# jzhoubu/vsearch

Hardware: AMD Instinct MI355X
Metric: queries/sec over 21M-doc sparse index, k=100; recall@100 vs reference (higher is better)
Workload: dtype f32

## Files before the change

vsearch_amd/csrc/bp_quad.h:

```cpp
#pragma once
#include "bp_walk.h"
#include "bp_quad_loop.h"
#include "bp_quad_asm.h"

#ifndef VS_QUAD_EPI
#define VS_QUAD_EPI 2
#endif

namespace vs {

constexpr int kQuadRows = 2048;
constexpr int kQuadQT = 8;
constexpr int kQuadPer = kBpEntCap / kScanThreads;
constexpr size_t kQuadAccBytes = (size_t)(kQuadRows / 16) * kQuadGroupDw * 4;
static_assert(kBpEntCap % kScanThreads == 0, "a thread owns a fixed number of entries");
static_assert(kQuadAccBytes >= kBpSortBytes, "the accumulator area holds the 8192-slot entry sort");
__host__ __device__ constexpr size_t quad_fixed_lds() { return kQuadAccBytes + (size_t)kBpCap * 8 + (size_t)kQuadQT * 16 + 64 * 4; }
__host__ __device__ constexpr size_t quad_cut_lds() { return quad_fixed_lds() + (size_t)(kBpEntCap + 64 + 64 * kQuadOverRead) * 8; }
__host__ __device__ constexpr size_t quad_lds_bytes() { return quad_cut_lds() + (size_t)kCutHistWords * 4; }
static_assert(quad_lds_bytes() <= (size_t)160 * 1024, "the quad walk's LDS");
static_assert(kBpCap == 2 * kScanThreads, "wg_cut_topk: two keys of the candidate buffer a thread");
static_assert(kQuadQT == 8 && (kQuadAccBytes + (size_t)kBpCap * 8) % 16 == 0, "the epilogue reads thresholds and counters 16 bytes at a time");
constexpr int kQuadListCap = 64 - 4 * kQuadOverRead, kQuadListBytes = (kQuadListCap + 4 * kQuadOverRead) * 8;
static_assert(kQuadListCap >= 16, "room for links in a wave's list");
static_assert(2 * kQuadListBytes * kScanWaves <= kBpCap * 8, "the link lists fit the sort buffer");
constexpr int kQuadLinked = kQuadCells - 2;
constexpr double kQuadMaxRatio = 3.0;
constexpr int kQuadPaceDefault = 0;
template <int CELLS, int LINKED>
__host__ __device__ constexpr uint32_t chunk_overflow(uint32_t n) { return n > (uint32_t)CELLS ? (n - (uint32_t)CELLS + (uint32_t)LINKED - 1u) / (uint32_t)LINKED : 0u; }
__host__ __device__ constexpr uint32_t quad_overflow_chunks(uint32_t n) { return chunk_overflow<kQuadCells, kQuadLinked>(n); }

template <int CELLS, int LINKED>
__global__ __launch_bounds__(kScanThreads) void quad_count_kernel(const uint32_t* pk_ptr, const uint4* cols, int64_t n_rows, int32_t n_cols, int32_t rows,
                                                                  uint32_t* dir, uint32_t* block_recs, unsigned long long* df_rec, unsigned long long* df_nnz,
                                                                  int32_t* overflow) {
    extern __shared__ __attribute__((aligned(16))) char smem[];
    uint32_t* cnt = reinterpret_cast<uint32_t*>(smem);
    __shared__ int scratch[32];
    const int tid = threadIdx.x;
    const int64_t n_blocks = (n_rows + rows - 1) / rows;
    const int seg = (n_cols + kScanThreads - 1) / kScanThreads;
    for (int64_t b = blockIdx.x; b < n_blocks; b += gridDim.x) {
        const int64_t r0 = b * rows, r1 = min(n_rows, r0 + rows);
        const uint32_t P0 = pk_ptr[r0], P1 = pk_ptr[r1];
        __syncthreads();
        for (int i = tid; i <= n_cols; i += kScanThreads) cnt[i] = 0;
        __syncthreads();
        for (uint32_t p = P0 + tid; p < P1; p += kScanThreads) {
            const uint4 cw = cols[p];
            const uint32_t cwv[4] = {cw.x, cw.y, cw.z, cw.w};
#pragma unroll
            for (int i = 0; i < 4; ++i) {
                atomicAdd(&cnt[cwv[i] & 0xFFFFu], 1u);
                atomicAdd(&cnt[cwv[i] >> 16], 1u);
            }
        }
        __syncthreads();
        const int i0 = min(n_cols, tid * seg), i1 = min(n_cols, i0 + seg);
        int mine = 0;
        for (int i = i0; i < i1; ++i) mine += (int)chunk_overflow<CELLS, LINKED>(cnt[i]);
        int tot = 0;
        int off = block_excl_scan(mine, scratch, tid, &tot);
        uint32_t* d = dir + (size_t)b * (n_cols + 1);
        for (int i = i0; i < i1; ++i) {
            const uint32_t c = cnt[i], r = chunk_overflow<CELLS, LINKED>(c);
            d[i] = bp_dir_pack((uint32_t)off, r);
            if (r > kBpDirRecMask || (uint32_t)off > kBpDirUnitMax) overflow[0] = 1;
            off += (int)r;
            atomicAdd(&df_rec[i], (unsigned long long)(1u + r));
            if (c) atomicAdd(&df_nnz[i], (unsigned long long)c);
        }
        if (tid == 0) { d[n_cols] = bp_dir_pack((uint32_t)tot, 0u); block_recs[b] = (uint32_t)n_cols + (uint32_t)tot; }
    }
}

template <int VS>
__global__ __launch_bounds__(kScanThreads) void quad_fill_kernel(const uint32_t* pk_ptr, const uint4* cols, const void* vals, int64_t n_rows, int32_t n_cols,
                                                                 int32_t rows, const uint32_t* dir, const unsigned long long* base, uint32_t* rec) {
    extern __shared__ __attribute__((aligned(16))) char smem[];
    uint32_t* cur = reinterpret_cast<uint32_t*>(smem);
    const int tid = threadIdx.x, lane = tid & 63, w = tid >> 6;
    const int64_t n_blocks = (n_rows + rows - 1) / rows;
    for (int64_t b = blockIdx.x; b < n_blocks; b += gridDim.x) {
        const int64_t r0 = b * rows, r1 = min(n_rows, r0 + rows);
        const uint32_t* d = dir + (size_t)b * (n_cols + 1);
        __syncthreads();
        for (int i = tid; i <= n_cols; i += kScanThreads) cur[i] = 0u;
        __syncthreads();
        uint32_t* brec = rec + (size_t)base[b] * kQuadCells;
        for (int64_t r = r0 + w; r < r1; r += kScanWaves) {
            const uint32_t p0 = pk_ptr[r], p1 = pk_ptr[r + 1];
            const uint32_t ai = quad_acc_index((uint32_t)(r - r0));
            for (uint32_t p = p0 + lane; p < p1; p += 64) {
                const uint4 cw = cols[p];
                const uint32_t cwv[4] = {cw.x, cw.y, cw.z, cw.w};
                uint32_t hb[8];
                if constexpr (VS == VM_F32) {
                    const float4* vp = reinterpret_cast<const float4*>(vals);
                    const float4 v0 = vp[2 * (size_t)p], v1 = vp[2 * (size_t)p + 1];
                    const float v[8] = {v0.x, v0.y, v0.z, v0.w, v1.x, v1.y, v1.z, v1.w};
#pragma unroll
                    for (int i = 0; i < 8; ++i) hb[i] = (uint32_t)__half_as_ushort(__float2half_rn(v[i]));
                } else {
                    const uint4 hv = reinterpret_cast<const uint4*>(vals)[p];
                    const uint32_t h4[4] = {hv.x, hv.y, hv.z, hv.w};
#pragma unroll
                    for (int i = 0; i < 8; ++i) hb[i] = (i & 1) ? (h4[i >> 1] >> 16) : (h4[i >> 1] & 0xFFFFu);
                }
#pragma unroll
// ... 36 lines not shown
        __syncthreads();
        for (int i = tid; i < nc * 16; i += 256) {
            const uint4 v = src[i];
            uint32_t* q = in + (i >> 4) * LD + (i & 15) * 4;
            q[0] = v.x; q[1] = v.y; q[2] = v.z; q[3] = v.w;
        }
        __syncthreads();
        if (tid < nc) {
            const uint32_t* mi = in + tid * LD;
            uint32_t* mo = out + tid * LD;
            uint32_t mask[4] = {0u, 0u, 0u, 0u}, fill[4] = {0u, 0u, 0u, 0u}, room[4] = {16u, 16u, 16u, 16u};
            const bool linked = (mi[63] >> 31) != 0u;
            if (linked) {
                mo[62] = mi[62]; mo[63] = mi[63];
                mask[2] |= 1u << (mi[62] & 31u); mask[3] |= 1u << (mi[63] & 31u);
                room[2] = 15u; room[3] = 15u;
            }
            for (int i = 0; i < (linked ? kQuadLinked : kQuadCells); ++i) {
                const uint32_t p = mi[i];
                if ((p & 0x7FFF0000u) == 0u) continue;
                const uint32_t bit = 1u << (p & 31u);
                int pick = -1, any = -1;
                uint32_t best = 17u, best_any = 17u;
#pragma unroll
                for (int j = 0; j < 4; ++j) {
                    if (fill[j] < room[j] && fill[j] < best_any) { best_any = fill[j]; any = j; }
                    if (fill[j] < room[j] && !(mask[j] & bit) && fill[j] < best) { best = fill[j]; pick = j; }
                }
                if (pick < 0) pick = any;
#pragma unroll
                for (int j = 0; j < 4; ++j)
                    if (j == pick) { mo[fill[j] * 4 + j] = p; mask[j] |= bit; ++fill[j]; }
            }
#pragma unroll
            for (int j = 0; j < 4; ++j)
                while (fill[j] < room[j]) {
                    const uint32_t freeb = ~mask[j];
                    const uint32_t bk = freeb ? (uint32_t)(__ffs((int)freeb) - 1) : 0u;
                    mo[fill[j] * 4 + j] = quad_acc_index(bk);
                    mask[j] |= 1u << bk;
                    ++fill[j];
                }
        }
        __syncthreads();
        uint4* dst = reinterpret_cast<uint4*>(rec + c0 * kQuadCells);
        for (int i = tid; i < nc * 16; i += 256) {
            const uint32_t* q = out + (i >> 4) * LD + (i & 15) * 4;
            dst[i] = make_uint4(q[0], q[1], q[2], q[3]);
        }
    }
}

typedef unsigned short quad_us2 __attribute__((ext_vector_type(2)));

static_assert(kQuadRows <= 2 * kScanThreads && kQuadQT * 2 <= 32, "a thread's filter bits: two document rounds x the slots in one word");
constexpr int kQuadFiltWords = kQuadRows / 32 + 1;
constexpr size_t kQuadFiltStageBytes = (size_t)kQuadFiltWords * kQuadQT * 4;
static_assert(kQuadFiltWords * kQuadQT <= kScanThreads && quad_lds_bytes() + kQuadFiltStageBytes <= (size_t)160 * 1024, "the per-query filter stage");
template <int TM, int FL = 0>
__global__ __launch_bounds__(kScanThreads) void bp_quad_topk(KArg<BpArgs, FL> a) {
    constexpr int QT = kQuadQT;
    extern __shared__ __attribute__((aligned(16))) char smem[];
    int32_t* acc = reinterpret_cast<int32_t*>(smem);
    uint64_t* sortbuf = reinterpret_cast<uint64_t*>(smem + kQuadAccBytes);
    unsigned long long* tau = reinterpret_cast<unsigned long long*>(sortbuf + kBpCap);
    unsigned long long* upper_sh = tau + QT;
    int* scratch = reinterpret_cast<int*>(upper_sh + QT);
    unsigned int* ccnt = reinterpret_cast<unsigned int*>(scratch + 48);
    unsigned int* chi = ccnt + QT;
    uint2* desc = reinterpret_cast<uint2*>(scratch + 64);
    const uint32_t desc_lds = (uint32_t)quad_fixed_lds();
    uint32_t* cut_hist = reinterpret_cast<uint32_t*>(smem + quad_cut_lds());

    const int tid = threadIdx.x, lane = tid & 63, wv = tid >> 6;
    const int K = a.k;
    uint64_t* my_gcand = a.gcand + (size_t)blockIdx.x * QT * kBpCap;
    const int64_t n_blocks = (a.n_rows + a.rows - 1) / a.rows;
    const int64_t items = (int64_t)(a.n_tiles_dev ? a.n_tiles_dev[0] : a.n_tiles) * a.nchunk;
    const unsigned long long k_rt0 = TM ? __builtin_amdgcn_s_memrealtime() : 0ull;
    auto lds_barrier = [&]() { asm volatile("s_waitcnt lgkmcnt(0)\n\ts_barrier" ::: "memory"); };
    const uint32_t list_a = (uint32_t)kQuadAccBytes + (uint32_t)wv * 2u * kQuadListBytes, list_b = list_a + kQuadListBytes;
    const uint32_t g8 = (uint32_t)(lane >> 4) * 8u, s16 = (uint32_t)(lane & 15) * 16u;

    for (int64_t item = blockIdx.x; item < items; item += gridDim.x) {
        const int tile = (int)(item / a.nchunk), c = (int)(item % a.nchunk);
        const int q0 = a.tiles[tile].x, nq = a.tiles[tile].y;
        [[maybe_unused]] long long tm = TM ? (long long)__builtin_readcyclecounter() : 0;
        [[maybe_unused]] uint32_t tacc[6] = {0u, 0u, 0u, 0u, 0u, 0u};
        auto lap = [&](int phase) {
            if constexpr (TM != 0) {
                const long long now = (long long)__builtin_readcyclecounter();
                tacc[phase] += (uint32_t)(now - tm);
                tm = now;
            }
        };
        const int64_t b0 = (int64_t)c * a.blocks_per_chunk, b1 = min(n_blocks, b0 + a.blocks_per_chunk);
        __syncthreads();
        const int64_t e0 = a.qptr[q0], e1 = a.qptr[q0 + nq];
        const int n_ent = (int)(e1 - e0);
        const int n_static = (n_ent + 63) & ~63;
        {
            uint64_t* skey = reinterpret_cast<uint64_t*>(acc);
            for (int i = tid; i < 8192; i += kScanThreads) {
                uint64_t key = 0;
                if (i < n_ent) {
                    const int64_t e = e0 + i;
                    int qs = 0;
                    while (e >= a.qptr[q0 + qs + 1]) ++qs;
                    const float w = a.qvals[e] * a.qscale[q0 + qs];
                    key = ((uint64_t)1 << 63) | ((uint64_t)(uint32_t)a.qcols[e] << 40) | ((uint64_t)qs << 32) | (uint64_t)__float_as_uint(w);
                }
                skey[i] = key;
            }
            wg_sort_desc<kScanThreads>(skey, 8192, tid);
            for (int i = tid; i < n_static + 64 * kQuadOverRead; i += kScanThreads) {
                uint2 dsc = make_uint2(0u, 0u);
                if (i < n_ent) {
                    const uint64_t key = skey[i];
                    const uint32_t col = (uint32_t)(key >> 40) & 0xFFFFu, qs = (uint32_t)(key >> 32) & 0xFFu;
                    dsc = make_uint2((col << 8) | (qs * 16u), (uint32_t)key);
                }
                desc[i] = dsc;
            }
            __syncthreads();
        }
        for (int i = tid; i < (int)(kQuadAccBytes / 4); i += kScanThreads) acc[i] = 0;
        if (tid < QT) { tau[tid] = 0ull; ccnt[tid] = 0u; chi[tid] = 0u; }
        if (tid < QT) upper_sh[tid] = (a.upper && tid < nq) ? a.upper[q0 + tid] : ~0ull;
        __syncthreads();
        const uint32_t trips = (uint32_t)(n_static / 64);
        bool pace_off = false;
        unsigned long long base_cur = b0 < b1 ? a.base[b0] : 0ull;
        for (int64_t b = b0; b < b1 || b == b0; ++b) {
            const bool have = b < b1;
            const int rows_b = have ? (int)min((int64_t)a.rows, a.n_rows - b * a.rows) : 0;
            [[maybe_unused]] uint32_t fw0 = 0u, fw1 = 0u;
            if constexpr (FL != 0) {
                if (a.filt.ld == 0) {
                    const uint64_t bit = (uint64_t)(a.filt.bit0 + b * a.rows + tid);
                    if (tid < rows_b) fw0 = a.filt.words[bit >> 5];
                    if (tid + kScanThreads < rows_b) fw1 = a.filt.words[(bit + kScanThreads) >> 5];
                } else if (have) {
                    const int64_t w0 = (a.filt.bit0 + b * a.rows) >> 5, w1 = (a.filt.bit0 + b * a.rows + rows_b - 1) >> 5;
                    const int q = tid & (QT - 1), w = tid / QT;
                    if (w < kQuadFiltWords && q < nq && w0 + w <= w1) fw0 = a.filt.words[(size_t)(q0 + q) * (size_t)a.filt.ld + (size_t)(w0 + w)];
                }
            }
            if (have && trips > 0) {
                const char* brec = a.rec + (size_t)base_cur * kQuadChunkBytes;
                auto chain = [&](uint32_t n, uint32_t cur, uint32_t nxt) {
                    for (int depth = 0; n > 0 && depth < kQuadRows / kQuadLinked + 2; ++depth) {
                        const uint32_t n_pad = (n + 3u) & ~3u;
                        if ((uint32_t)lane < n_pad - n + 4u * kQuadOverRead)
                            reinterpret_cast<uint2*>(smem + cur)[n + (uint32_t)lane] = make_uint2(0u, 0u);
                        asm volatile("s_waitcnt lgkmcnt(0)" ::: "memory");
                        n = quad_list_asm(cur + g8, n_pad / 4u, brec, s16, nxt, (uint32_t)kQuadListCap);
                        const uint32_t t = cur; cur = nxt; nxt = t;
                    }
                };
                const uint32_t n_link = quad_walk_asm(desc_lds + (uint32_t)wv * 32u + g8, trips, brec, s16, list_a, (uint32_t)kQuadListCap);
                if (n_link <= (uint32_t)kQuadListCap) {
                    chain(n_link, list_a, list_b);
                } else {
                    constexpr uint32_t kSeg = kQuadListCap / 4;
                    for (uint32_t t0 = 0; t0 < trips; t0 += kSeg) {
                        const uint32_t n = quad_collect_asm(desc_lds + (uint32_t)wv * 32u + g8 + t0 * 512u, min(kSeg, trips - t0), brec, s16, list_a, (uint32_t)kQuadListCap);
                        chain(n, list_a, list_b);
                    }
                }
            }
            lap(1);
            if (a.pace && items <= (int64_t)gridDim.x && tid == 0 && have && !pace_off) {
                uint32_t* pc = a.pace + (size_t)c * a.blocks_per_chunk;
                const int64_t rel = b - b0;
                if (!((a.knob & 64) && blockIdx.x == 0))
                    __hip_atomic_fetch_add(pc + rel, 1u, __ATOMIC_RELAXED, __HIP_MEMORY_SCOPE_AGENT);
                if (rel >= a.pace_window) {
                    const uint32_t need = (uint32_t)(items / a.nchunk);
                    if (!pace_wait(pc + rel - a.pace_window, need)) pace_off = true;
                }
            }
            if (b + 1 < b1) base_cur = a.base[b + 1];
            if (a.gtau && tid < nq) { const unsigned long long g = a.gtau[q0 + tid]; if (g > tau[tid]) tau[tid] = g; }
            [[maybe_unused]] uint32_t fbits = 0u;
            [[maybe_unused]] uint32_t* fstage = reinterpret_cast<uint32_t*>(smem + quad_lds_bytes());
            if constexpr (FL != 0) {
                if (a.filt.ld == 0) {
#pragma unroll
                    for (int r = 0; r < 2; ++r) {
                        const uint64_t bit = (uint64_t)(a.filt.bit0 + b * a.rows + r * kScanThreads + tid);
                        if (r * kScanThreads + tid < rows_b && (((r ? fw1 : fw0) >> (bit & 31u)) & 1u)) fbits |= 0xFFu << (r * QT);
                    }
                } else if (tid < kQuadFiltWords * QT) {
                    fstage[tid] = fw0;
                }
                __builtin_amdgcn_s_waitcnt(0x0F70);
            }
            lds_barrier();
            if constexpr (FL != 0) {
                if (a.filt.ld != 0) {
                    const int64_t w0 = (a.filt.bit0 + b * a.rows) >> 5;
#pragma unroll
                    for (int r = 0; r < 2; ++r) {
                        const int d = r * kScanThreads + tid;
                        if (d < rows_b) {
                            const uint64_t bit = (uint64_t)(a.filt.bit0 + b * a.rows + d);
                            const uint4* p = reinterpret_cast<const uint4*>(fstage + ((int64_t)(bit >> 5) - w0) * QT);
                            const uint4 lo = p[0], hi = p[1];
                            const uint32_t w[QT] = {lo.x, lo.y, lo.z, lo.w, hi.x, hi.y, hi.z, hi.w};
#pragma unroll
                            for (int q = 0; q < QT; ++q) fbits |= ((w[q] >> (bit & 31u)) & 1u) << (r * QT + q);
                        }
                    }
                }
            }
            uint32_t pf = 0;
            if ((a.knob & 512) == 0 && b + 1 < b1 && (uint32_t)(lane >> 3) < trips) {
                const uint32_t dx = *reinterpret_cast<const uint32_t*>(smem + desc_lds + (uint32_t)(lane >> 3) * 512u + (uint32_t)wv * 32u + (uint32_t)((lane >> 1) & 3) * 8u);
                const char* pl = a.rec + (size_t)base_cur * kQuadChunkBytes + (dx & 0xFFFFFF00u) + (uint32_t)(lane & 1) * 128u;
                asm volatile("global_load_dword %0, %1, off" : "=v"(pf) : "v"(pl) : "memory");
            }
            lap(2);
            int32_t thr[QT];
            bool thr_stale = true;
            for (int d0 = 0; d0 < rows_b || d0 == 0; d0 += kScanThreads) {
                const int d = d0 + tid;
                const bool more = d0 + kScanThreads < rows_b;
                const uint32_t inc = more ? 1u : 0x10000u;
                if (d0 == 0 || thr_stale) {
                    const uint4* t4 = reinterpret_cast<const uint4*>(tau);
#pragma unroll
                    for (int i = 0; i < QT / 2; ++i) {
                        const uint4 t = t4[i];
                        thr[2 * i] = 2 * i < nq ? (int32_t)(t.y ^ 0x80000000u) : 0x7FFFFFFF;
                        thr[2 * i + 1] = 2 * i + 1 < nq ? (int32_t)(t.w ^ 0x80000000u) : 0x7FFFFFFF;
                    }
                    thr_stale = false;
                }
                if (d < rows_b) {
                    const int64_t row = b * a.rows + d;
                    int32_t sums[QT];
#if VS_QUAD_EPI == 0
                    int32_t* pa = acc + quad_acc_index((uint32_t)d);
#pragma unroll
                    for (int q = 0; q < QT; ++q) sums[q] = pa[q * 16];
#pragma unroll
                    for (int q = 0; q < QT; ++q) pa[q * 16] = 0;
#elif VS_QUAD_EPI == 1
                    {
                        const uint32_t pa = quad_acc_index((uint32_t)d) * 4u, zero = 0u;
                        asm volatile("ds_wrxchg_rtn_b32 %0, %8, %9\n\tds_wrxchg_rtn_b32 %1, %8, %9 offset:64\n\tds_wrxchg_rtn_b32 %2, %8, %9 offset:128\n\t"
                                     "ds_wrxchg_rtn_b32 %3, %8, %9 offset:192\n\tds_wrxchg_rtn_b32 %4, %8, %9 offset:256\n\tds_wrxchg_rtn_b32 %5, %8, %9 offset:320\n\t"
                                     "ds_wrxchg_rtn_b32 %6, %8, %9 offset:384\n\tds_wrxchg_rtn_b32 %7, %8, %9 offset:448\n\ts_waitcnt lgkmcnt(0)"
                                     : "=&v"(sums[0]), "=&v"(sums[1]), "=&v"(sums[2]), "=&v"(sums[3]), "=&v"(sums[4]), "=&v"(sums[5]), "=&v"(sums[6]), "=&v"(sums[7])
                                     : "v"(pa), "v"(zero) : "memory");
                    }
#else
                    {
                        const uint32_t pa = quad_acc_index((uint32_t)d) * 4u, zero = 0u;
                        unsigned long long s01, s23, s45, s67;
                        asm volatile("ds_wrxchg2_rtn_b32 %0, %4, %5, %5 offset0:0 offset1:16\n\tds_wrxchg2_rtn_b32 %1, %4, %5, %5 offset0:32 offset1:48\n\t"
                                     "ds_wrxchg2_rtn_b32 %2, %4, %5, %5 offset0:64 offset1:80\n\tds_wrxchg2_rtn_b32 %3, %4, %5, %5 offset0:96 offset1:112\n\ts_waitcnt lgkmcnt(0)"
                                     : "=&v"(s01), "=&v"(s23), "=&v"(s45), "=&v"(s67) : "v"(pa), "v"(zero) : "memory");
                        sums[0] = (int32_t)(uint32_t)s01; sums[1] = (int32_t)(uint32_t)(s01 >> 32); sums[2] = (int32_t)(uint32_t)s23; sums[3] = (int32_t)(uint32_t)(s23 >> 32);
                        sums[4] = (int32_t)(uint32_t)s45; sums[5] = (int32_t)(uint32_t)(s45 >> 32); sums[6] = (int32_t)(uint32_t)s67; sums[7] = (int32_t)(uint32_t)(s67 >> 32);
                    }
#endif
#pragma unroll
                    for (int q = 0; q < QT; ++q) {
                        if (sums[q] >= thr[q] && (FL == 0 || ((fbits >> ((d0 >= kScanThreads ? QT : 0) + q)) & 1u) != 0u)) {
                            const uint32_t hi = (uint32_t)sums[q] ^ 0x80000000u;
                            const uint64_t key = ((uint64_t)hi << 32) | (uint32_t)(~(uint32_t)row);
                            if (key > tau[q] && key < upper_sh[q]) {
                                const uint32_t old = atomicAdd(&ccnt[q], inc);
                                my_gcand[(size_t)q * kBpCap + (old & 0xFFFFu) + (old >> 16)] = key;
                            }
                        }
                    }
                }
                static_assert(kQuadRows <= 2 * kScanThreads, "the cut counter has two fields, first rounds | last round: a block is at most two epilogue rounds");
                lds_barrier();
                if ((a.knob & 128) && __builtin_amdgcn_readfirstlane(wv) == 5)
                    for (int i = 0; i < (a.knob >> 12); ++i) __builtin_amdgcn_s_sleep(8);
                const bool last = b + 1 >= b1 && !more;
                uint32_t cmax;
                {
                    const uint4* c4 = reinterpret_cast<const uint4*>(ccnt);
                    const uint4 c0 = c4[0], c1 = c4[1];
                    const uint32_t w[QT] = {c0.x, c0.y, c0.z, c0.w, c1.x, c1.y, c1.z, c1.w};
                    uint32_t t[QT];
                    if (more) {
                        const uint4 h0 = c4[2], h1 = c4[3];
                        const uint32_t h[QT] = {h0.x, h0.y, h0.z, h0.w, h1.x, h1.y, h1.z, h1.w};
#pragma unroll
                        for (int q = 0; q < QT; ++q) t[q] = __builtin_amdgcn_udot2(__builtin_bit_cast(quad_us2, w[q]), quad_us2{1, 0}, h[q], false);
                    } else {
#pragma unroll
                        for (int q = 0; q < QT; ++q) t[q] = __builtin_amdgcn_udot2(__builtin_bit_cast(quad_us2, w[q]), quad_us2{1, 1}, 0u, false);
                        if (tid < QT) chi[tid] = ccnt[tid] >> 16;
                    }
                    cmax = max(max(max(t[0], t[1]), max(t[2], t[3])), max(max(t[4], t[5]), max(t[6], t[7])));
                }
                const bool any = last || cmax > (uint32_t)(kBpCap - kScanThreads);
                [[maybe_unused]] long long t_cut = 0;
                if constexpr (TM != 0) t_cut = (long long)__builtin_readcyclecounter();
                if (any) __syncthreads();
                thr_stale = any;
                if (any)
                for (int qs = 0; qs < nq; ++qs) {
                    const uint32_t cw = ccnt[qs], cnt = (cw & 0xFFFFu) + (more ? chi[qs] : (cw >> 16));
                    if (last || cnt > (uint32_t)(kBpCap - kScanThreads)) {
                        for (int i = tid; i < kBpCap; i += kScanThreads) sortbuf[i] = (uint32_t)i < cnt ? my_gcand[(size_t)qs * kBpCap + i] : 0ull;
                        if (last) {
                            uint64_t* out = a.cand + ((size_t)(q0 + qs) * a.nchunk + c) * (size_t)K;
                            if (K <= 256) {
                                wg_final_topk256<kScanThreads>(sortbuf, cnt, K, my_gcand + (size_t)qs * kBpCap, out, cut_hist, tid);
                            } else {
                                wg_sort_desc<kScanThreads>(sortbuf, kBpCap, tid);
                                for (int i = tid; i < K; i += kScanThreads) out[i] = sortbuf[i];
                            }
                        } else if (cnt > (uint32_t)K) {
                            const unsigned long long kth_sel = wg_cut_topk<kScanThreads>(sortbuf, K, my_gcand + (size_t)qs * kBpCap, cut_hist, tid);
                            if (tid == 0) {
                                const unsigned long long kth = kth_sel;
                                if (kth > tau[qs]) tau[qs] = kth;
                                if (a.gtau && kth != 0ull) atomicMax(a.gtau + q0 + qs, kth);
                                ccnt[qs] = (uint32_t)K;
                                chi[qs] = 0u;
                            }
                        }
                        __syncthreads();
                    }
                }
                if constexpr (TM != 0) { if (any) tacc[3] += (uint32_t)((long long)__builtin_readcyclecounter() - t_cut); }
            }
            asm volatile("s_waitcnt vmcnt(0)" : "+v"(pf) : : "memory");
            lap(4);
            if constexpr (TM != 0) tacc[5] += 1u;
            if (b + 1 >= b1) break;
        }
        if constexpr (TM != 0) {
            if ((tid & 63) == 0) {
#pragma unroll
                for (int i = 0; i < 6; ++i) atomicAdd(a.timing + i, (unsigned long long)tacc[i]);
            }
        }
    }
    if (TM && threadIdx.x == 0) {
        a.timing[16 + 4 * blockIdx.x] = __builtin_amdgcn_s_memrealtime() - k_rt0;
        a.timing[17 + 4 * blockIdx.x] = k_rt0;
        a.timing[18 + 4 * blockIdx.x] = (unsigned long long)__builtin_amdgcn_s_getreg((3 << 11) | 20);
        a.timing[19 + 4 * blockIdx.x] = (unsigned long long)__builtin_amdgcn_s_getreg((31 << 11) | 4);
    }
}

}
```

vsearch_amd/csrc/bp_search.hip:

```cpp
#include "csr_internal.h"
#include "bp_refine.h"
#include "bp_bin.h"
#include "bp_quad.h"
#include "bp_head.h"
#include "bp_bq.h"

#include <chrono>
#include <vector>

namespace vs {


bool bp_wanted(const vs_index* idx) {
    if (idx->bp_pref == 0 || idx->n_rows <= 0 || idx->n_packets <= 0) return false;
    if (((size_t)idx->n_cols + 1) * 4 + 4096 > 160 * 1024) return false;
    if (idx->bp_pref == 1) return true;
    if (idx->store_dtype == VS_NONE) return idx->n_rows >= 65536;
    return idx->n_rows >= 16384 && (double)idx->nnz / (double)idx->n_rows >= 256.0;
}

void bp_release(vs_index* idx) {
    idx->bp_dir.release(); idx->bp_base.release(); idx->bp_rec.release(); idx->bp_df.release(); idx->bp_vmax.release();
    idx->bp_hmap.release(); idx->bp_strip.release();
    idx->bp_n_head = 0;
// ... 436 lines not shown
                       bq_pk ? idx->bp_bq_maxrow : 0, bq_pk ? flag16 : (uint32_t*)nullptr);
    if (bq_pk) hipLaunchKernelGGL(bq_split_kernel<0>, dim3(1), dim3(kScanThreads), 0, s, (const int2*)tiles, reinterpret_cast<const int32_t*>(dplan), (const uint32_t*)flag16,
                                  tiles16, tiles2, n_split);
    VS_HIP(hipGetLastError());
    VS_STAGE("sparsify", s);
    const bool head_gemm = idx->bp_n_head > 0 && idx->bp_head_gemm;
    int tiles_per_pass = 0, n_pass = 1;
    const int head_ks = bp_head_pad(idx->bp_n_head) / 32;
    if (head_gemm) {
        const size_t per_tile = (size_t)n_blocks * (size_t)idx->bp_rows * 8 * 2;
        size_t free_b = 0, total_b = 0;
        VS_HIP(hipMemGetInfo(&free_b, &total_b));
        DevBuf& head_out = device_scratch(idx->device, kScratchHeadOut);
        DevBuf& head_w = device_scratch(idx->device, kScratchHeadW);
        const size_t have = head_out.bytes, margin = (size_t)6 << 30;
        const size_t room = std::min<size_t>(free_b + have > margin ? free_b + have - margin : 0, total_b / 4);
        static const int tpp_env = getenv("VS_HEAD_TILES") ? atoi(getenv("VS_HEAD_TILES")) : 0;
        int tpp = (int)std::min<size_t>(std::max<size_t>(have, std::min<size_t>(room, (size_t)48 << 30)) / std::max<size_t>(per_tile, 1), (size_t)ceil_div(B, qt));
        if (tpp_env > 0) tpp = std::min(tpp, tpp_env);
        if (idx->bp_head_tiles > 0) tpp = std::min(tpp, idx->bp_head_tiles);
        if (tpp >= 64) tpp = tpp / 64 * 64;
        else if (tpp >= 2) tpp &= ~1;
        if (tpp < 1) return fail(VS_ENOMEM, "head pre-pass: no HBM for the dense sums of one tile (%.2f GB)", (double)per_tile / 1e9);
        tiles_per_pass = tpp;
        VS_TRY(head_out.reserve((size_t)tpp * per_tile));
        VS_TRY(head_w.reserve((size_t)((tpp + 1) / 2) * head_ks * 1024));
        n_pass = ceil_div(B, tpp);
    }
    const int n_tiles_est = head_gemm ? std::min(tiles_per_pass, ceil_div(B, qt)) : ceil_div(B, qt);
    const int nchunk = bp_choose_chunks(idx, n_tiles_est, n_blocks, plan.nchunk);
    const int nchunk_fb = (int)std::min<int64_t>(n_blocks, 64);
    const int grid = (int)std::min<int64_t>((int64_t)B * nchunk, idx->cu_count);
    VS_TRY(idx->ws_mq_cand.reserve((size_t)idx->cu_count * kQT * std::max(kBpCap, kFlCap) * 8));
    VS_TRY(idx->ws_cand.reserve(std::max((size_t)B * nchunk * kp, (size_t)B * nchunk_fb * k) * 8));
    BpArgs a{};
    a.rows = idx->bp_rows;
    a.dir = idx->bp_dir.as<uint32_t>();
    a.al_shift = idx->bp_al_shift;
    a.base = idx->bp_base.as<unsigned long long>();
    a.rec = idx->bp_rec.as<char>();
    a.n_rows = idx->n_rows;
    a.n_cols = V;
    a.k = kp;
    a.nchunk = nchunk;
    a.blocks_per_chunk = ceil_div64(n_blocks, nchunk);
    a.qptr = qptr;
    a.qcols = qcols;
    a.qvals = qvals;
    a.tiles = tiles;
    a.n_tiles = 0;
    a.n_tiles_dev = reinterpret_cast<const int32_t*>(dplan);
    a.ent_cap = vals_cap;
    a.cand = idx->ws_cand.as<uint64_t>();
    a.gcand = idx->ws_mq_cand.as<uint64_t>();
    a.qscale = qscale;
    a.gtau = gtau;
    const bool fl = idx->filt.words != nullptr;
    a.df = idx->bp_df.p ? idx->bp_df.as<unsigned long long>() + V : nullptr;
    a.hmap = idx->bp_n_head > 0 ? idx->bp_hmap.as<uint16_t>() : nullptr;
    a.strip = idx->bp_strip.as<__half>();
    a.n_head = idx->bp_n_head;
    if (a.n_head > 0) {
        int ve;
        (void)frexpf(idx->bp_vmax_f, &ve);
        a.head_pre = ldexpf(1.f, ve - 16);
        a.head_mul = ldexpf(1.f, 16 - ve);
    }
    idx->last_path = 3;
    idx->last_plan_dev = dplan;
    idx->last_split_dev = bq_pk ? n_split : nullptr;
    idx->last_plan_rs = idx->bp_quad ? kQuadChunkBytes : idx->bp_bq ? kBqChunkBytes : bp_rec_bytes(bp_record_vm(idx));
    idx->last_plan_blocks = n_blocks;
    static const int pace_env = getenv("VS_BP_PACE") ? atoi(getenv("VS_BP_PACE")) : -1;
    const bool bin_walk = idx->store_dtype == VS_NONE && idx->bp_walk_pref != 0 && !idx->bp_bq;
    const int pace_w = pace_env >= 0 ? pace_env : (idx->bp_pace >= 0 ? idx->bp_pace : (idx->bp_bq ? kBqPaceDefault : bin_walk ? 32 : (idx->bp_quad ? kQuadPaceDefault : 0)));
    if (pace_w > 0) {
        VS_TRY(idx->ws_pace.reserve((size_t)nchunk * a.blocks_per_chunk * 4));
        VS_HIP(hipMemsetAsync(idx->ws_pace.p, 0, (size_t)nchunk * a.blocks_per_chunk * 4, s));
        a.pace = idx->ws_pace.as<uint32_t>();
        a.pace_window = pace_w;
    }
    static const int knob_env = getenv("VS_BP_KNOB") ? atoi(getenv("VS_BP_KNOB")) : 0;
    a.knob = knob_env;
    static const bool timing_on = getenv("VS_BP_TIMING") != nullptr;
    DevBuf timing;
    if (timing_on) {
        VS_TRY(timing.alloc(128 + (size_t)grid * 32));
        VS_HIP(hipMemsetAsync(timing.p, 0, 128 + (size_t)grid * 32, s));
        a.timing = timing.as<unsigned long long>();
    }
    for (int pass = 0; pass < n_pass; ++pass) {
        if (head_gemm) {
            HeadArgs h{};
            h.strip = a.strip;
            h.wt = device_scratch(idx->device, kScratchHeadW).as<uint4>();
            h.out = device_scratch(idx->device, kScratchHeadOut).as<uint16_t>();
            h.tiles = tiles;
            h.n_tiles_dev = a.n_tiles_dev;
            h.tile0 = pass * tiles_per_pass;
            h.tile_cnt = tiles_per_pass;
            h.qptr = qptr; h.qcols = qcols; h.qvals = qvals; h.qscale = qscale;
            h.hmap = a.hmap;
            h.n_head = a.n_head;
            h.rows = idx->bp_rows;
            h.n_rows = idx->n_rows;
            h.n_blocks = n_blocks;
            h.head_pre = a.head_pre; h.head_mul = ldexpf(a.head_mul, -kHeadOutShift);
            a.head_out = h.out;
            a.tile0 = h.tile0;
            a.tile_cnt = tiles_per_pass;
            if (a.pace && pass > 0) VS_HIP(hipMemsetAsync(idx->ws_pace.p, 0, (size_t)nchunk * a.blocks_per_chunk * 4, s));
            ProfScope prof("head_gemm", s);
            hipLaunchKernelGGL(head_weights_kernel<0>, dim3(tiles_per_pass), dim3(256), 0, s, h);
            static const int shape_env = getenv("VS_HEAD_SHAPE") ? atoi(getenv("VS_HEAD_SHAPE")) : 0;
            const bool ring = shape_env == 222 || (shape_env == 0 && (idx->bp_head_product == 1 || (idx->bp_head_product < 0 && tiles_per_pass >= 32 && idx->cu_count % 8 == 0)));
            if (ring) {
                VS_HIP(hipFuncSetAttribute((const void*)head_gemm_lds_kernel<0>, hipFuncAttributeMaxDynamicSharedMemorySize, 163840));
                hipLaunchKernelGGL(head_gemm_lds_kernel<0>, dim3(idx->cu_count), dim3(256), 163840, s, h);
            } else if (shape_env == 24) hipLaunchKernelGGL((head_gemm_kernel<2, 4>), dim3(idx->cu_count), dim3(512), 0, s, h);
            else hipLaunchKernelGGL((head_gemm_kernel<1, 4, 1>), dim3(idx->cu_count), dim3(256), 0, s, h);
            VS_HIP(hipGetLastError());
        }
        ProfScope prof("csr_scan_topk", s);
        if (bq_pk) {
            BpArgs a16 = a, a2 = a;
            a16.tiles = tiles16; a16.n_tiles_dev = n_split;
            a2.tiles = tiles2; a2.n_tiles_dev = n_split + 1;
            const size_t lds = bq_lds_bytes(2);
            if (vals_cap > kBqEntCap) return fail(VS_EUNSUPPORTED, "bag-of-token chunks: tile entries beyond the table");
            VS_TRY(fl ? launch_bq_split<1>(idx, a16, a2, grid, lds, s) : launch_bq_split<0>(idx, a16, a2, grid, lds, s));
            VS_HIP(hipGetLastError());
        } else
        VS_TRY((launch_bp_walk<kQT, AM_FIX>(idx, a, grid, vals_cap, s)));
    }
    if (timing_on) {
        unsigned long long h[16] = {0};
        VS_HIP(hipMemcpyAsync(h, timing.p, 128, hipMemcpyDeviceToHost, s));
        VS_HIP(hipStreamSynchronize(s));
        {
            std::vector<unsigned long long> wg((size_t)grid * 4);
            VS_HIP(hipMemcpy(wg.data(), timing.as<unsigned long long>() + 16, wg.size() * 8, hipMemcpyDeviceToHost));
            double tmin = 1e30, tmax = 0, tsum = 0;
            double xs[8] = {0}, xc[8] = {0}, xn[8] = {0};
            unsigned long long s_min = ~0ull, s_max = 0, e_max = 0;
            for (int i = 0; i < grid; ++i) {
                const double t = (double)wg[4 * i] * 1e-5, cyc = (double)wg[4 * i + 1];
                tmin = std::min(tmin, t); tmax = std::max(tmax, t); tsum += t;
                const int x = (int)(wg[4 * i + 2] & 7);
                xs[x] += t; xc[x] += cyc; xn[x] += 1;
                s_min = std::min(s_min, wg[4 * i + 1]); s_max = std::max(s_max, wg[4 * i + 1]); e_max = std::max(e_max, wg[4 * i + 1] + wg[4 * i]);
            }
            fprintf(stderr, "[vsearch_hip] walk: workgroup time min %.2f mean %.2f max %.2f ms; starts spread over %.2f ms, first start -> last end %.2f ms;", tmin, tsum / grid, tmax,
                    (double)(s_max - s_min) * 1e-5, (double)(e_max - s_min) * 1e-5);
            fprintf(stderr, "\n");
            if (getenv("VS_BP_TIMING_WG")) {
                std::vector<int> ord(grid);
                for (int i = 0; i < grid; ++i) ord[i] = i;
                std::sort(ord.begin(), ord.end(), [&](int x, int y) { return wg[4 * x] > wg[4 * y]; });
                for (int j = 0; j < std::min(grid, 12); ++j) {
                    const int i = ord[j];
                    const unsigned hw = (unsigned)wg[4 * i + 3];
                    fprintf(stderr, "   wg %3d: %.2f ms, %.1f Mcycles, xcc %d se %d sh %d cu %d simd %d\n", i, (double)wg[4 * i] * 1e-5, (double)wg[4 * i + 1] * 1e-6, (int)(wg[4 * i + 2] & 7),
                            (hw >> 13) & 7, (hw >> 12) & 1, (hw >> 8) & 15, (hw >> 4) & 3);
                }
            }
        }
        if (idx->bp_quad) {
            const double bw = (double)std::max<unsigned long long>(1, h[5]);
            fprintf(stderr, "[vsearch_hip] quad walk, cycles per block and wave: gathers back %.0f, scan %.0f, barrier %.0f, emit %.0f, barrier (+ rest of the plan) %.0f\n", (double)h[6] / bw, (double)h[7] / bw,
                    (double)h[8] / bw, (double)h[9] / bw, (double)h[3] / bw);
            h[12] = h[14] = 0;
        }
        if (h[12] | h[14]) {
            const double bw = (double)std::max<unsigned long long>(1, h[5]) / 16.0;
            fprintf(stderr, "[vsearch_hip] binary walk, cycles per block: wave 0 walk %.0f wait %.0f; wave 8 walk %.0f wait %.0f\n", (double)h[12] / bw, (double)h[13] / bw,
                    (double)h[14] / bw, (double)h[15] / bw);
        }
        const double tot = (double)(h[0] + h[1] + h[2] + h[3] + h[4]);
        fprintf(stderr, "[vsearch_hip] walk wave-cycles: prologue %.1f %%, list walk %.1f %%, barrier wait %.1f %%, dense %.1f %%, epilogue %.1f %%; per block and wave: "
                        "walk %.0f wait %.0f dense %.0f epilogue %.0f cycles\n", 100.0 * h[0] / tot, 100.0 * h[1] / tot, 100.0 * h[2] / tot, 100.0 * h[3] / tot, 100.0 * h[4] / tot,
                (double)h[1] / (double)std::max<unsigned long long>(1, h[5]), (double)h[2] / (double)std::max<unsigned long long>(1, h[5]),
                (double)h[3] / (double)std::max<unsigned long long>(1, h[5]), (double)h[4] / (double)std::max<unsigned long long>(1, h[5]));
    }
    VS_STAGE("filter walk", s);
    RefineArgs r{};
    r.cand = a.cand;
    r.n_cand = (int64_t)nchunk * kp;
    r.run_len = kp;
    r.B = B; r.k = k; r.kp = kp;
    r.pk_ptr = idx->pk_ptr.as<uint32_t>();
    r.cols = idx->cols.as<uint4>();
    r.vals = idx->vals.p;
    r.n_cols = V;
    r.n_rows = idx->n_rows;
    r.q = dq;
    r.qscale = qscale;
    r.qslack = qslack;
    r.qwsum = qwsum;
    r.quant = (idx->bp_quant || idx->bp_n_head > 0) ? 1 : 0;
    if (head_gemm) r.quant = 2;
    r.force_flag = idx->bp_force_fb ? 1 : 0;
    r.id_offset = id_offset;
    r.out_ids = d_ids;
    r.out_scores = d_scores;
    r.out_ld = out_ld;
    r.flags = flags;
    {
        ProfScope prof("refine_topk", s);
        const bool img = refine_lds_bytes(V, 1) <= (size_t)160 * 1024;
        const size_t rlds = refine_lds_bytes(V, img ? 1 : 0);
        const int rgrid = std::min(B, idx->cu_count * (img ? 1 : 2));
        void (*rk)(RefineArgs) = idx->store_dtype == VS_F32 ? (img ? refine_topk_kernel<VM_F32, 1> : refine_topk_kernel<VM_F32, 0>)
                               : idx->store_dtype == VS_F16 ? (img ? refine_topk_kernel<VM_F16, 1> : refine_topk_kernel<VM_F16, 0>)
                                                            : (img ? refine_topk_kernel<VM_BIN, 1> : refine_topk_kernel<VM_BIN, 0>);
        if (fl) rk = idx->store_dtype == VS_F32 ? (img ? refine_topk_kernel<VM_F32, 1, 1> : refine_topk_kernel<VM_F32, 0, 1>)
                   : idx->store_dtype == VS_F16 ? (img ? refine_topk_kernel<VM_F16, 1, 1> : refine_topk_kernel<VM_F16, 0, 1>)
                                                : (img ? refine_topk_kernel<VM_BIN, 1, 1> : refine_topk_kernel<VM_BIN, 0, 1>);
        VS_HIP(hipFuncSetAttribute((const void*)rk, hipFuncAttributeMaxDynamicSharedMemorySize, (int)rlds));
        hipLaunchKernelGGL(rk, dim3(rgrid), dim3(kScanThreads), rlds, s, r);
        VS_HIP(hipGetLastError());
    }
    VS_STAGE("refine", s);
    {
        ProfScope prof("exact_fallback", s);
        hipLaunchKernelGGL(fb_plan_kernel<0>, dim3(1), dim3(kScanThreads), 0, s, flags, B, fb_tiles, fb_n);
        ScanArgs sa{};
        sa.pk_ptr = idx->pk_ptr.as<uint32_t>();
        sa.cols = idx->cols.as<uint4>();
        sa.vals = idx->vals.p;
        sa.q = dq;
        sa.n_rows = idx->n_rows;
        sa.n_cols = V;
        sa.B = B;
        sa.k = k;
        sa.nchunk = nchunk_fb;
        sa.rows_per_chunk = ceil_div64(idx->n_rows, nchunk_fb);
        sa.cand = a.cand;
        VS_TRY(fl ? launch_exact_scan<1>(idx, sa, fb_tiles, fb_n, s) : launch_exact_scan<0>(idx, sa, fb_tiles, fb_n, s));
        MergeArgs m{};
        m.cand = a.cand;
        m.n_cand = (int64_t)nchunk_fb * k;
        m.B = B;
        m.k = k;
        m.id_offset = id_offset;
        m.out_ids = d_ids;
        m.out_scores = d_scores;
        m.out_ld = out_ld;
        m.col0 = 0;
        m.run_len = k;
        m.sel = fb_tiles;
        m.sel_n = fb_n;
        hipLaunchKernelGGL((fl ? merge_topk_kernel<1> : merge_topk_kernel<0>), dim3(std::min(B, idx->cu_count)), dim3(kScanThreads), 0, s, m);
        VS_HIP(hipGetLastError());
// ... 12 lines not shown
```

vsearch_amd/csrc/bp_walk.h:

```cpp
#pragma once
#include <hip/hip_runtime.h>
#include <hip/hip_fp16.h>
#include <stdint.h>
#include <type_traits>

#include "csr_scan.h"
#include "dense_csr.h"

namespace vs {

enum : int { AM_F64 = 0, AM_FIX = 1 };

constexpr int kBpRowsMax = 2048;
constexpr int kBpRowsMaxBin = 2048;
constexpr int kBpCap = 2048;
constexpr int kBpMaxK = kBpCap - kScanThreads;
constexpr int kFlCap = 4096;
constexpr int kBpEntCap = 7168;
constexpr int kBpNB = 4;
constexpr int kBpNBWide = 6;
constexpr size_t kBpSortBytes = (size_t)8192 * 8;

__host__ __device__ constexpr int bp_rec_bytes(int vm) { return vm == VM_F32 ? 48 : (vm == VM_F16 ? 32 : 16); }
__host__ __device__ constexpr int bp_align_shift(int vm) { return vm == VM_F32 ? 3 : (vm == VM_F16 ? 2 : 0); }
// ... 256 lines not shown
                    }
                }
                for (int j = 0; j < R; ++j) {
                    uint4 iw;
                    iw.x = oid[j * 8 + 0] | ((uint32_t)oid[j * 8 + 1] << 16); iw.y = oid[j * 8 + 2] | ((uint32_t)oid[j * 8 + 3] << 16);
                    iw.z = oid[j * 8 + 4] | ((uint32_t)oid[j * 8 + 5] << 16); iw.w = oid[j * 8 + 6] | ((uint32_t)oid[j * 8 + 7] << 16);
                    *reinterpret_cast<uint4*>(rp + (size_t)j * RS) = iw;
                    if constexpr (VM == VM_F16) {
                        uint4 vw;
                        vw.x = oval[j * 8 + 0] | (oval[j * 8 + 1] << 16); vw.y = oval[j * 8 + 2] | (oval[j * 8 + 3] << 16);
                        vw.z = oval[j * 8 + 4] | (oval[j * 8 + 5] << 16); vw.w = oval[j * 8 + 6] | (oval[j * 8 + 7] << 16);
                        *reinterpret_cast<uint4*>(rp + (size_t)j * RS + 16) = vw;
                    } else {
                        *reinterpret_cast<uint4*>(rp + (size_t)j * RS + 16) = make_uint4(oval[j * 8 + 0], oval[j * 8 + 1], oval[j * 8 + 2], oval[j * 8 + 3]);
                        *reinterpret_cast<uint4*>(rp + (size_t)j * RS + 32) = make_uint4(oval[j * 8 + 4], oval[j * 8 + 5], oval[j * 8 + 6], oval[j * 8 + 7]);
                    }
                }
            }
        }
    }
}

template <int UNUSED>
__global__ __launch_bounds__(kScanThreads) void bp_walk_kernel(const uint32_t* colfreq, const unsigned long long* df_rec, const unsigned long long* df_nnz,
                                                               int32_t n_cols, int64_t* out) {
    __shared__ unsigned long long red[2][kScanThreads / 64];
    unsigned long long v = 0, z = 0;
    for (int c = threadIdx.x; c < n_cols; c += kScanThreads) { v += (unsigned long long)colfreq[c] * df_rec[c]; z += (unsigned long long)colfreq[c] * df_nnz[c]; }
    for (int o = 32; o > 0; o >>= 1) { v += __shfl_xor(v, o, 64); z += __shfl_xor(z, o, 64); }
    if ((threadIdx.x & 63) == 0) { red[0][threadIdx.x >> 6] = v; red[1][threadIdx.x >> 6] = z; }
    __syncthreads();
    if (threadIdx.x == 0) {
        unsigned long long t = 0, u = 0;
        for (int i = 0; i < kScanThreads / 64; ++i) { t += red[0][i]; u += red[1][i]; }
        out[0] = (int64_t)t;
        out[1] = (int64_t)u;
    }
}

constexpr int kPaceSpins = 1 << 14;
__device__ __forceinline__ bool pace_wait(const uint32_t* p, uint32_t need) {
    for (int spins = 0; spins < kPaceSpins; ++spins) {
        if (__hip_atomic_load(p, __ATOMIC_RELAXED, __HIP_MEMORY_SCOPE_AGENT) >= need) return true;
        __builtin_amdgcn_s_sleep(8);
    }
    return false;
}

typedef unsigned short walk_us2 __attribute__((ext_vector_type(2)));

struct BpArgs {
    int32_t rows;
    const uint32_t* dir;
    int32_t al_shift;
    const unsigned long long* base;
    const char* rec;
    int64_t n_rows;
    int32_t n_cols;
    int32_t k;
    int32_t nchunk;
    int64_t blocks_per_chunk;
    const int64_t* qptr;
    const int32_t* qcols;
    const float* qvals;
    const int2* tiles;
    int32_t n_tiles;
    const int32_t* n_tiles_dev;
    int32_t ent_cap;
    uint64_t* cand;
    uint64_t* gcand;
    const uint64_t* upper;
    const unsigned long long* df;
    unsigned long long* gtau;
    const float* qscale;
    const uint16_t* hmap;
    const __half* strip;
    int32_t n_head;
    float head_pre, head_mul;
    const uint16_t* head_out;
    int32_t tile0, tile_cnt;
    uint32_t* pace;
    int32_t pace_window;
    int32_t knob;
    unsigned long long* debug;
    unsigned long long* timing;
};

template <int QT, int AM, int RMAX>
__host__ __device__ constexpr size_t bp_acc_bytes() { return (((size_t)(RMAX + 1) * (QT + 1) * (AM == AM_F64 ? 8 : 4)) + 15) & ~(size_t)15; }
__host__ __device__ inline size_t bp_head_lds(int n_head) { return n_head > 0 ? (size_t)16 * (bp_head_pad(n_head) + 8) * 2 : 0; }
template <int QT, int AM, int RMAX>
__host__ __device__ inline size_t bp_lds_bytes(int ent_cap, int n_head = 0) {
    return bp_acc_bytes<QT, AM, RMAX>() + (size_t)kBpCap * 8 + (size_t)QT * 16 + 64 * 4 + (size_t)kCutHistWords * 4 + (size_t)ent_cap * 8 + bp_head_lds(n_head);
}

__device__ __forceinline__ uint64_t make_key_fix(int32_t a, uint32_t row) {
    return ((uint64_t)((uint32_t)a ^ 0x80000000u) << 32) | (uint32_t)(~row);
}
__device__ __forceinline__ int32_t key_fix(uint64_t k) { return (int32_t)((uint32_t)(k >> 32) ^ 0x80000000u); }

__device__ __forceinline__ uint32_t acc_off_lo(uint32_t idw, uint32_t pitch, uint32_t so) {
    uint32_t r;
    asm("v_mad_u32_u16 %0, %1, %2, %3" : "=v"(r) : "v"(idw), "v"(pitch), "v"(so));
    return r;
}
__device__ __forceinline__ uint32_t acc_off_hi(uint32_t idw, uint32_t pitch, uint32_t so) {
    uint32_t r;
    asm("v_mad_u32_u16 %0, %1, %2, %3 op_sel:[1,0,0,0]" : "=v"(r) : "v"(idw), "v"(pitch), "v"(so));
    return r;
}

typedef uint32_t u32x4 __attribute__((ext_vector_type(4)));
__device__ __forceinline__ void load_rec48(u32x4& a, u32x4& b, u32x4& c, uint32_t off, unsigned long long base) {
    asm volatile("global_load_dwordx4 %0, %3, %4\n\tglobal_load_dwordx4 %1, %3, %4 offset:16\n\tglobal_load_dwordx4 %2, %3, %4 offset:32"
                 : "=&v"(a), "=&v"(b), "=&v"(c) : "v"(off), "s"(base));
}
__device__ __forceinline__ void load_rec32(u32x4& a, u32x4& b, uint32_t off, unsigned long long base) {
    asm volatile("global_load_dwordx4 %0, %2, %3\n\tglobal_load_dwordx4 %1, %2, %3 offset:16" : "=&v"(a), "=&v"(b) : "v"(off), "s"(base));
}
__device__ __forceinline__ void load_rec16(u32x4& a, uint32_t off, unsigned long long base) {
    asm volatile("global_load_dwordx4 %0, %1, %2" : "=&v"(a) : "v"(off), "s"(base));
}
#define VS_WAIT_CASES(OPS)                                                                                              \
    switch (n) {                                                                                                        \
        case 1: asm volatile("s_waitcnt vmcnt(1)" : OPS); break;                                                      \
        case 2: asm volatile("s_waitcnt vmcnt(2)" : OPS); break;                                                      \
        case 3: asm volatile("s_waitcnt vmcnt(3)" : OPS); break;                                                      \
        case 4: asm volatile("s_waitcnt vmcnt(4)" : OPS); break;                                                      \
        case 5: asm volatile("s_waitcnt vmcnt(5)" : OPS); break;                                                      \
        case 6: asm volatile("s_waitcnt vmcnt(6)" : OPS); break;                                                      \
        case 7: asm volatile("s_waitcnt vmcnt(7)" : OPS); break;                                                      \
        case 8: asm volatile("s_waitcnt vmcnt(8)" : OPS); break;                                                      \
        case 9: asm volatile("s_waitcnt vmcnt(9)" : OPS); break;                                                      \
        case 10: asm volatile("s_waitcnt vmcnt(10)" : OPS); break;                                                    \
        case 11: asm volatile("s_waitcnt vmcnt(11)" : OPS); break;                                                    \
        case 12: asm volatile("s_waitcnt vmcnt(12)" : OPS); break;                                                    \
        case 13: asm volatile("s_waitcnt vmcnt(13)" : OPS); break;                                                    \
        case 14: asm volatile("s_waitcnt vmcnt(14)" : OPS); break;                                                    \
        case 15: asm volatile("s_waitcnt vmcnt(15)" : OPS); break;                                                    \
        case 16: asm volatile("s_waitcnt vmcnt(16)" : OPS); break;                                                    \
        case 17: asm volatile("s_waitcnt vmcnt(17)" : OPS); break;                                                    \
        case 18: asm volatile("s_waitcnt vmcnt(18)" : OPS); break;                                                    \
        case 19: asm volatile("s_waitcnt vmcnt(19)" : OPS); break;                                                    \
        case 20: asm volatile("s_waitcnt vmcnt(20)" : OPS); break;                                                    \
        case 21: asm volatile("s_waitcnt vmcnt(21)" : OPS); break;                                                    \
        case 22: asm volatile("s_waitcnt vmcnt(22)" : OPS); break;                                                    \
        case 23: asm volatile("s_waitcnt vmcnt(23)" : OPS); break;                                                    \
        case 24: asm volatile("s_waitcnt vmcnt(24)" : OPS); break;                                                    \
        default: asm volatile("s_waitcnt vmcnt(0)" : OPS); break;                                                       \
    }
#define VS_OPS3 "+v"(a), "+v"(b), "+v"(c)
#define VS_OPS2 "+v"(a), "+v"(b)
#define VS_OPS1 "+v"(a)
__device__ __forceinline__ void wait_loads(int n, u32x4& a, u32x4& b, u32x4& c) { VS_WAIT_CASES(VS_OPS3) }
__device__ __forceinline__ void wait_loads(int n, u32x4& a, u32x4& b) { VS_WAIT_CASES(VS_OPS2) }
__device__ __forceinline__ void wait_loads(int n, u32x4& a) { VS_WAIT_CASES(VS_OPS1) }
#undef VS_OPS1
#undef VS_OPS2
#undef VS_OPS3
#undef VS_WAIT_CASES
__device__ __forceinline__ void lds_add(uint32_t addr, int32_t v) {
    __hip_atomic_fetch_add(reinterpret_cast<__attribute__((address_space(3))) int32_t*>(addr), v, __ATOMIC_RELAXED, __HIP_MEMORY_SCOPE_WORKGROUP);
}
__device__ __forceinline__ void lds_add(uint32_t addr, double v) {
    __hip_atomic_fetch_add(reinterpret_cast<__attribute__((address_space(3))) double*>(addr), v, __ATOMIC_RELAXED, __HIP_MEMORY_SCOPE_WORKGROUP);
}
// ... 492 lines not shown
```

Before: 7998.

## Split next-block record prefetch cooperatively across blocks sharing an XCD

Adds a cooperative prefetch mode for the quad walk. When every work item has its own block, the blocks on the same XCD (8 XCDs assumed) each touch an interleaved, strided subset of the next block's 128-byte record lines, up to a configurable line count. This is meant to warm the shared L2 for the whole next block, where before each wave only prefetched the lines its own descriptors named. It costs extra global loads per block and may fetch lines that are never used. It also depends on the blockIdx-to-XCD mapping holding.

```diff
diff --git a/vsearch_amd/csrc/bp_quad.h b/vsearch_amd/csrc/bp_quad.h
--- a/vsearch_amd/csrc/bp_quad.h
+++ b/vsearch_amd/csrc/bp_quad.h
@@ -26,6 +26,7 @@
 static_assert(2 * kQuadListBytes * kScanWaves <= kBpCap * 8, "the link lists fit the sort buffer");
 constexpr int kQuadLinked = kQuadCells - 2;
 constexpr double kQuadMaxRatio = 3.0;
+constexpr int kQuadPfLines = 384;
 constexpr int kQuadPaceDefault = 0;
 template <int CELLS, int LINKED>
 __host__ __device__ constexpr uint32_t chunk_overflow(uint32_t n) { return n > (uint32_t)CELLS ? (n - (uint32_t)CELLS + (uint32_t)LINKED - 1u) / (uint32_t)LINKED : 0u; }
@@ -228,6 +229,12 @@
     const uint32_t list_a = (uint32_t)kQuadAccBytes + (uint32_t)wv * 2u * kQuadListBytes, list_b = list_a + kQuadListBytes;
     const uint32_t g8 = (uint32_t)(lane >> 4) * 8u, s16 = (uint32_t)(lane & 15) * 16u;
 
+    uint32_t pf_r = 0u, pf_R = 0u;
+    if (a.pf_xcds > 0 && items <= (int64_t)gridDim.x && (int64_t)blockIdx.x < items) {
+        const uint32_t X = (uint32_t)a.pf_xcds, R = ((uint32_t)items - blockIdx.x % X + X - 1u) / X;
+        if (R >= 2u) { pf_r = blockIdx.x / X; pf_R = R; }
+    }
+    [[maybe_unused]] uint32_t n_coop = 0u;
     for (int64_t item = blockIdx.x; item < items; item += gridDim.x) {
         const int tile = (int)(item / a.nchunk), c = (int)(item % a.nchunk);
         const int q0 = a.tiles[tile].x, nq = a.tiles[tile].y;
@@ -361,10 +368,19 @@
                 }
             }
             uint32_t pf = 0;
-            if ((a.knob & 512) == 0 && b + 1 < b1 && (uint32_t)(lane >> 3) < trips) {
-                const uint32_t dx = *reinterpret_cast<const uint32_t*>(smem + desc_lds + (uint32_t)(lane >> 3) * 512u + (uint32_t)wv * 32u + (uint32_t)((lane >> 1) & 3) * 8u);
-                const char* pl = a.rec + (size_t)base_cur * kQuadChunkBytes + (dx & 0xFFFFFF00u) + (uint32_t)(lane & 1) * 128u;
-                asm volatile("global_load_dword %0, %1, off" : "=v"(pf) : "v"(pl) : "memory");
+            if ((a.knob & 512) == 0 && b + 1 < b1 && trips > 0) {
+                if (pf_R != 0u) {
+                    const uint32_t L = pf_r + pf_R * (uint32_t)tid;
+                    if (tid < a.pf_lines && L < 2u * (uint32_t)a.n_cols) {
+                        const char* pl = a.rec + (size_t)base_cur * kQuadChunkBytes + (size_t)L * 128u;
+                        asm volatile("global_load_dword %0, %1, off" : "=v"(pf) : "v"(pl) : "memory");
+                    }
+                    if constexpr (TM != 0) n_coop += 1u;
+                } else if ((uint32_t)(lane >> 3) < trips) {
+                    const uint32_t dx = *reinterpret_cast<const uint32_t*>(smem + desc_lds + (uint32_t)(lane >> 3) * 512u + (uint32_t)wv * 32u + (uint32_t)((lane >> 1) & 3) * 8u);
+                    const char* pl = a.rec + (size_t)base_cur * kQuadChunkBytes + (dx & 0xFFFFFF00u) + (uint32_t)(lane & 1) * 128u;
+                    asm volatile("global_load_dword %0, %1, off" : "=v"(pf) : "v"(pl) : "memory");
+                }
             }
             lap(2);
             int32_t thr[QT];
@@ -493,6 +509,7 @@
         }
     }
     if (TM && threadIdx.x == 0) {
+        if (n_coop) atomicAdd(a.timing + 10, (unsigned long long)n_coop);
         a.timing[16 + 4 * blockIdx.x] = __builtin_amdgcn_s_memrealtime() - k_rt0;
         a.timing[17 + 4 * blockIdx.x] = k_rt0;
         a.timing[18 + 4 * blockIdx.x] = (unsigned long long)__builtin_amdgcn_s_getreg((3 << 11) | 20);
diff --git a/vsearch_amd/csrc/bp_search.hip b/vsearch_amd/csrc/bp_search.hip
--- a/vsearch_amd/csrc/bp_search.hip
+++ b/vsearch_amd/csrc/bp_search.hip
@@ -542,6 +542,11 @@
     }
     static const int knob_env = getenv("VS_BP_KNOB") ? atoi(getenv("VS_BP_KNOB")) : 0;
     a.knob = knob_env;
+    static const int pf_env = getenv("VS_BP_PF_LINES") ? atoi(getenv("VS_BP_PF_LINES")) : 0;
+    if (idx->bp_quad && idx->cu_count % 8 == 0 && 8 % nchunk == 0 && !(knob_env & 1024)) {
+        a.pf_xcds = 8;
+        a.pf_lines = std::min(pf_env > 0 ? pf_env : kQuadPfLines, kScanThreads);
+    }
     static const bool timing_on = getenv("VS_BP_TIMING") != nullptr;
     DevBuf timing;
     if (timing_on) {
@@ -627,8 +632,8 @@
         }
         if (idx->bp_quad) {
             const double bw = (double)std::max<unsigned long long>(1, h[5]);
-            fprintf(stderr, "[vsearch_hip] quad walk, cycles per block and wave: gathers back %.0f, scan %.0f, barrier %.0f, emit %.0f, barrier (+ rest of the plan) %.0f\n", (double)h[6] / bw, (double)h[7] / bw,
-                    (double)h[8] / bw, (double)h[9] / bw, (double)h[3] / bw);
+            fprintf(stderr, "[vsearch_hip] quad walk, cycles per block and wave: gathers back %.0f, scan %.0f, barrier %.0f, emit %.0f, barrier (+ rest of the plan) %.0f; prefetch %s\n", (double)h[6] / bw,
+                    (double)h[7] / bw, (double)h[8] / bw, (double)h[9] / bw, (double)h[3] / bw, (a.knob & 512) ? "none" : h[10] ? "coop" : "wave");
             h[12] = h[14] = 0;
         }
         if (h[12] | h[14]) {
diff --git a/vsearch_amd/csrc/bp_walk.h b/vsearch_amd/csrc/bp_walk.h
--- a/vsearch_amd/csrc/bp_walk.h
+++ b/vsearch_amd/csrc/bp_walk.h
@@ -362,6 +362,8 @@
     uint32_t* pace;
     int32_t pace_window;
     int32_t knob;
+    int32_t pf_xcds;
+    int32_t pf_lines;
     unsigned long long* debug;
     unsigned long long* timing;
 };
```

Measured after the change: 8095, median of 6. 1.2% higher.
